# Twilight-Dream-Of-Magic/KolmogorovLike-DataCompressor

Hardware: AMD Instinct MI355X
Metric: compress MB/s at fixed block size, bit-exact vs reference; 1/2/4/8-GPU scaling (higher is better)
Workload: dtype u8; 1 GPU; enwik-style synthetic text (kolm.datagen.enwik_like, seed 20251212+rank), 256 MiB per GPU resident in HBM, 1 MiB fixed blocks, candidates 0..8 + MDL, payloads emitted in HBM; block_size=1048576, bytes_per_gpu=268435456, blocks_per_gpu=256, parallelism=block-shard x1

## Files before the change

### kolmogorovlike-datacompressor_amd/csrc/k_lsd.hip

```cpp
#include "kolm_internal.h"

#include <algorithm>
#include <cstdlib>
#include <string>
#include <vector>

namespace kolm {

namespace {

#ifndef KOLM_LSD_T
#define KOLM_LSD_T 4096
#endif
constexpr u32 LSD_T = KOLM_LSD_T;
constexpr u32 LSD_PT = LSD_T / WG;
static_assert(LSD_PT % 4 == 0 && LSD_PT <= 32, "head masks hold 32 slots per thread");

struct LsdGeom {
    Geom geo;
    u32 tpb;
    const u8* text;
    const u8* FEd;
    Factors fac;
    __device__ inline bool range(u32 t, u32& lo, u32& hi, u32& b) const {
        b = t / tpb;
        const u32 k = t - b * tpb;
        lo = geo.base(b) + k * LSD_T;
        const u32 e = geo.end(b);
        hi = min(lo + LSD_T, e);
        return lo < e;
    }
};

template <int P>
__device__ inline u32 digit(u32 key) {
    return (key >> (8 * P)) & 255u;
}

__device__ inline void load16(const u32* X, u32 i0, u32 hi, u32 (&v)[LSD_PT]) {
    if ((i0 & 3) == 0 && i0 + LSD_PT <= hi) {
        const uint4* p = reinterpret_cast<const uint4*>(X + i0);
#pragma unroll
        for (int q = 0; q < (int)LSD_PT / 4; ++q) {
            const uint4 t = p[q];
            v[4 * q] = t.x;
            v[4 * q + 1] = t.y;
            v[4 * q + 2] = t.z;
            v[4 * q + 3] = t.w;
        }
    } else {
#pragma unroll
        for (u32 e = 0; e < LSD_PT; ++e) v[e] = i0 + e < hi ? X[i0 + e] : 0u;
    }
// ... 505 lines not shown
    u32 len[LSD_PT];
    u32 nseg = 0;
#pragma unroll
    for (int e = LSD_PT - 1; e >= 0; --e) {
        const u32 i = i0 + e;
        len[e] = 0;
        if (hd[e]) {
            len[e] = nh - i;
            nh = i;
            nseg += len[e] >= 2;
        }
    }
    const u32 incl = wave_incl_scan(nseg, OpAddU(), 0u);
    if (lane == 63) sh3[w] = incl;
    if (split) anysplit = 1;
    __syncthreads();
    u32 off = incl - nseg;
    for (u32 q = 0; q < w; ++q) off += sh3[q];
    if (tid == WG - 1) {
        const u32 tot = off + nseg;
        wbase = tot ? atomicAdd(next_cnt, tot) : 0u;
        if (anysplit) blk_split[b] = 1;
    }
    __syncthreads();
    off += wbase;
#pragma unroll
    for (u32 e = 0; e < LSD_PT; ++e)
        if (len[e] >= 2) next[off++] = Seg{i0 + e, len[e]};
}

__global__ __launch_bounds__(WG) void k_r0_rk(Geom geo, u32 nwin, const u32* PP, u32* RK) {
    __shared__ u32 win[R0_WIN];
    const u32 b = blockIdx.x / nwin, k = blockIdx.x - b * nwin;
    const u32 base = geo.base(b), e = geo.end(b);
    const u32 lo = base + k * R0_WIN;
    if (lo >= e) return;
    const u32 n = min(R0_WIN, e - lo);
    for (u32 d = threadIdx.x; d < n; d += WG) {
        const u32 v = PP[lo + d];
        win[v >> 20] = base + (v & 0xFFFFFu);
    }
    __syncthreads();
    if ((lo & 3) == 0 && (n & 1023) == 0) {
        uint4* dst = reinterpret_cast<uint4*>(RK + lo);
        const uint4* src = reinterpret_cast<const uint4*>(win);
        for (u32 i = threadIdx.x; i < n / 4; i += WG) dst[i] = src[i];
    } else {
        for (u32 i = threadIdx.x; i < n; i += WG) RK[lo + i] = win[i];
    }
}

constexpr u32 AL_PER = 65536;

__global__ __launch_bounds__(WG) void k_alpha_present(Geom geo, const u8* text, u32 parts, u32* pres) {
    __shared__ u32 f[256];
    f[threadIdx.x] = 0;
    __syncthreads();
    const u32 b = blockIdx.x / parts, part = blockIdx.x - b * parts;
    const u32 lo = geo.base(b) + part * AL_PER, hi = min(lo + AL_PER, geo.end(b));
    for (u32 i = lo + threadIdx.x; i < hi; i += WG) f[text[i]] = 1u;
    __syncthreads();
    const u64 m = __ballot(f[threadIdx.x] != 0);
    if ((threadIdx.x & 31) == 0) {
        const u32 word = (u32)(m >> (threadIdx.x & 32));
        if (word) atomicOr(&pres[(u64)b * 8 + (threadIdx.x >> 5)], word);
    }
}

__global__ __launch_bounds__(WG) void k_alpha_codes(const u32* pres, u8* code, u32* wmax) {
    __shared__ u32 pw[8];
    const u32 b = blockIdx.x, c = threadIdx.x;
    if (c < 8) pw[c] = pres[(u64)b * 8 + c];
    __syncthreads();
    u32 r = 0;
    for (u32 k = 0; k < (c >> 5); ++k) r += __popc(pw[k]);
    r += __popc(pw[c >> 5] & ((1u << (c & 31)) - 1u));
    code[(u64)b * 256 + c] = (u8)r;
    if (c == 255) {
        const u32 sigma = r + ((pw[7] >> 31) & 1u);
        const u32 w = sigma > 1 ? 32 - __clz(sigma - 1) : 1u;
        atomicMax(wmax, w);
    }
}

__global__ __launch_bounds__(WG) void k_keypos_r0(LsdGeom g, const u8* code, u32 C, u32 w, u32 sh, u32* KA, u32* KB,
                                                  u32* hist0,
                                                  ScanParts sp = ScanParts{}, u32 part = 0) {
    __shared__ __align__(16) u8 tx[LSD_T + 64];
    __shared__ u8 cd[256];
    __shared__ TileCounts h0;
    u32 lo, hi, b;
    const u32 tile = xcd_tile();
    if (!g.range(tile, lo, hi, b)) {
        if (hist0) hist0[(u64)tile * 256 + threadIdx.x] = 0;
        return;
    }
    if (hist0) h0.clear();
    const u32 N = (u32)g.geo.N;
    cd[threadIdx.x] = code[(u64)b * 256 + threadIdx.x];
    const u32 n = min(hi + C + (part ? 1u : 0u), N) - lo;
    if ((((uintptr_t)g.text + lo) & 3) == 0) {
        const u32* src = reinterpret_cast<const u32*>(g.text + lo);
        u32* dst = reinterpret_cast<u32*>(tx);
        for (u32 i = threadIdx.x; i < (n + 3) / 4; i += WG) dst[i] = src[i];
    } else {
        for (u32 i = threadIdx.x; i < n; i += WG) tx[i] = g.text[lo + i];
    }
    __syncthreads();
    const u32 i0 = threadIdx.x * LSD_PT;
    if (lo + i0 < hi) {
    u8 fed[LSD_PT];
    if (((lo + i0) & 15) == 0 && lo + i0 + LSD_PT <= hi) {
#pragma unroll
        for (u32 q = 0; q < LSD_PT / 16; ++q) {
            const uint4 v = reinterpret_cast<const uint4*>(g.FEd + lo + i0)[q];
            const u32 wd[4] = {v.x, v.y, v.z, v.w};
#pragma unroll
            for (u32 e = 0; e < 16; ++e) fed[16 * q + e] = (u8)(wd[e >> 2] >> (8 * (e & 3)));
        }
    } else {
#pragma unroll
        for (u32 e = 0; e < LSD_PT; ++e) fed[e] = lo + i0 + e < hi ? g.FEd[lo + i0 + e] : (u8)255;
    }
    const u64 mask = C * w >= 64 ? ~0ull : ((1ull << (C * w)) - 1);
    u64 key = 0;
    for (u32 k = 0; k < C; ++k) key = (key << w) | (i0 + k < n ? cd[tx[i0 + k]] : 0u);
    u32 ka[LSD_PT], kb[LSD_PT];
    const u32 psh = w - part, plo = sh - part;
#pragma unroll
    for (u32 e = 0; e < LSD_PT; ++e) {
        const u32 x = i0 + e + C;
        const u32 nc = x < n ? cd[tx[x]] : 0u;
        const u64 kk = (key << sh) | (part ? (u64)(nc >> psh) << plo : 0ull);
        ka[e] = (u32)kk;
        kb[e] = (u32)(kk >> 32);
        key = ((key << w) | nc) & mask;
    }
    const u32 need = C + (part ? 1u : 0u);
#pragma unroll
    for (u32 e = 0; e < LSD_PT; ++e) {
        const u32 p = lo + i0 + e;
        if (p < hi && fed[e] < need) {
            u32 fs, m;
            g.fac.locate(g.geo, p, fs, m);
            u32 t = p - fs;
            u64 k2 = 0;
            for (u32 k = 0; k < C; ++k) {
                k2 = (k2 << w) | cd[g.text[fs + t]];
                if (++t == m) t = 0;
            }
            const u64 kk = (k2 << sh) | (part ? (u64)(cd[g.text[fs + t]] >> psh) << plo : 0ull);
            ka[e] = (u32)kk;
            kb[e] = (u32)(kk >> 32);
        }
    }
    const u32 p0 = lo + i0;
    if ((p0 & 3) == 0 && p0 + LSD_PT <= hi) {
#pragma unroll
        for (u32 q = 0; q < LSD_PT / 4; ++q) {
            reinterpret_cast<uint4*>(KA + p0)[q] = make_uint4(ka[4 * q], ka[4 * q + 1], ka[4 * q + 2], ka[4 * q + 3]);
            if (KB) reinterpret_cast<uint4*>(KB + p0)[q] = make_uint4(kb[4 * q], kb[4 * q + 1], kb[4 * q + 2], kb[4 * q + 3]);
        }
    } else {
        for (u32 e = 0; e < LSD_PT && p0 + e < hi; ++e) {
            KA[p0 + e] = ka[e];
            if (KB) KB[p0 + e] = kb[e];
        }
    }
    if (hist0) {
#pragma unroll
        for (u32 e = 0; e < LSD_PT; ++e)
            if (p0 + e < hi) h0.add(digit<0>(ka[e]));
    }
    }
    if (hist0) {
        __syncthreads();
        const u32 v = h0.total(threadIdx.x);
        hist0[(u64)tile * 256 + threadIdx.x] = v;
        add_part_total(g, sp, tile, v);
    }
}

template <int P, int SRC, int G, int OUT>
void lsd_pass(const LsdGeom& g, u32 nt, const u32* kin, const u32* pin, u32* kout, u32* pout, const u32* kg,
              u32* hist, bool counted, hipStream_t s, KTimer* kt, const ScanParts& sp) {
    static const std::string hn = "k_lsd_hist<" + std::to_string(P) + ", " + std::to_string(SRC) + ">";
    static const std::string sn = "k_lsd_scatter_w<" + std::to_string(P) + ", " + std::to_string(SRC) + ", " +
                                  std::to_string(G) + (OUT ? ", " + std::to_string(OUT) + ">" : std::string(">"));
    const u64 N = g.geo.N, H = (u64)nt * 1024;
    if (!counted) {
        KScope k(kt, KT_LSD, hn.c_str(), (SRC == SRC_REC ? 8 : 4) * N + H);
        k_lsd_hist<P, SRC><<<nt, WG, 0, s>>>(g, kin, hist, sp);
    }
    if (sp.cur) {
        KScope k(kt, KT_LSD, "k_lsd_scan2", 2 * H);
        k_lsd_scan2<<<g.geo.nb * sp.np, WG, 0, s>>>(g, hist, sp);
    } else {
        KScope k(kt, KT_LSD, "k_lsd_scan", 3 * H);
        static const int s4e = getenv("KOLM_LSD_SCAN4") ? atoi(getenv("KOLM_LSD_SCAN4")) : -1;
        const int mode = s4e >= 0 ? s4e : (g.geo.nb < 64 ? 1 : 0);
        if (mode == 1)
            k_lsd_scanp<4><<<g.geo.nb, 4 * WG, 0, s>>>(g, hist);
        else if (mode == 2)
            k_lsd_scanp<2><<<g.geo.nb, 2 * WG, 0, s>>>(g, hist);
        else
            k_lsd_scan<<<g.geo.nb, WG, 0, s>>>(g, hist);
    }
    {
        const u64 in = (SRC == SRC_PAIR || SRC == SRC_REC) ? 8 : 4, outb = OUT == OUT_PK ? 4 : 8;
        KScope k(kt, KT_LSD, sn.c_str(), (in + outb) * N + (G ? 4 * N : 0) + H);
        k_lsd_scatter_w<P, SRC, G, OUT><<<nt, WG, 0, s>>>(g, kin, pin, kout, pout, kg, hist);
    }
}

void run_pass_rec(u32 idx, const LsdGeom& g, u32 nt, const u32* kin, u32* kout, u32* pout, const u32* kg,
                  u32* hist, hipStream_t s, KTimer* kt, const ScanParts& sp) {
    switch (idx) {
        case 0: return lsd_pass<0, SRC_KP, 0, OUT_REC>(g, nt, kin, nullptr, kout, nullptr, nullptr, hist, true, s, kt, sp);
        case 1: return lsd_pass<1, SRC_REC, 0, OUT_REC>(g, nt, kin, nullptr, kout, nullptr, nullptr, hist, false, s, kt, sp);
        case 2: return lsd_pass<2, SRC_REC, 0, OUT_PK>(g, nt, kin, nullptr, kout, nullptr, nullptr, hist, false, s, kt, sp);
        case 3: return lsd_pass<3, SRC_PK, 1, OUT_REC>(g, nt, kin, nullptr, kout, nullptr, kg, hist, false, s, kt, sp);
        case 4: return lsd_pass<0, SRC_REC, 0, OUT_REC>(g, nt, kin, nullptr, kout, nullptr, nullptr, hist, false, s, kt, sp);
        case 5: return lsd_pass<1, SRC_REC, 0, OUT_REC>(g, nt, kin, nullptr, kout, nullptr, nullptr, hist, false, s, kt, sp);
        case 6: return lsd_pass<2, SRC_REC, 0, OUT_REC>(g, nt, kin, nullptr, kout, nullptr, nullptr, hist, false, s, kt, sp);
        default: return lsd_pass<3, SRC_REC, 0, OUT_PAIR>(g, nt, kin, nullptr, kout, pout, nullptr, hist, false, s, kt, sp);
    }
}

using PassFn = void (*)(const LsdGeom&, u32, const u32*, const u32*, u32*, u32*, const u32*, u32*, bool, hipStream_t,
                        KTimer*, const ScanParts&);
template <int P>
constexpr PassFn pass_of(int src_kp, int gat) {
    return src_kp ? (gat ? lsd_pass<P, SRC_KP, 1, 0> : lsd_pass<P, SRC_KP, 0, 0>)
                  : (gat ? lsd_pass<P, SRC_PAIR, 1, 0> : lsd_pass<P, SRC_PAIR, 0, 0>);
}
void run_pass(int P, bool src_kp, bool gat, const LsdGeom& g, u32 nt, const u32* kin, const u32* pin, u32* kout,
              u32* pout, const u32* kg, u32* hist, bool counted, hipStream_t s, KTimer* kt, int pk,
              const ScanParts& sp) {
    if (pk == 1) return lsd_pass<2, SRC_PAIR, 0, OUT_PK>(g, nt, kin, pin, kout, pout, kg, hist, counted, s, kt, sp);
    if (pk == 2) return lsd_pass<3, SRC_PK, 1, OUT_PAIR>(g, nt, kin, pin, kout, pout, kg, hist, counted, s, kt, sp);
    const int a = src_kp ? 1 : 0, c = gat ? 1 : 0;
    const PassFn f = P == 0 ? pass_of<0>(a, c) : P == 1 ? pass_of<1>(a, c) : P == 2 ? pass_of<2>(a, c) : pass_of<3>(a, c);
    f(g, nt, kin, pin, kout, pout, kg, hist, counted, s, kt, sp);
}

}

u32 lsd_tiles(const Geom& geo) { return (geo.bs + LSD_T - 1) / LSD_T * geo.nb; }

u32 launch_alpha(const Geom& geo, const u8* text, u32* pres, u8* code, u32* d_w, u32* h_w, bool compact,
                 hipStream_t s, KTimer* kt) {
    if (!geo.N) return 8;
    if (!compact) {
        std::vector<u8> id(256 * (size_t)geo.nb);
        for (size_t i = 0; i < id.size(); ++i) id[i] = (u8)i;
        KOLM_HIP_CHECK(hipMemcpyAsync(code, id.data(), id.size(), hipMemcpyHostToDevice, s));
        KOLM_HIP_CHECK(hipStreamSynchronize(s));
        return 8;
    }
    launch_alpha_async(geo, text, pres, code, d_w, h_w, s, kt);
    KOLM_HIP_CHECK(hipStreamSynchronize(s));
    return alpha_width(*h_w);
}

void launch_alpha_async(const Geom& geo, const u8* text, u32* pres, u8* code, u32* d_w, u32* h_w, hipStream_t s,
                        KTimer* kt, bool zeroed) {
    if (!geo.N) {
        if (h_w) *h_w = 8;
        return;
    }
    const u32 parts = (geo.bs + AL_PER - 1) / AL_PER;
    if (!zeroed) {
        KOLM_HIP_CHECK(hipMemsetAsync(pres, 0, sizeof(u32) * 8 * geo.nb, s));
        KOLM_HIP_CHECK(hipMemsetAsync(d_w, 0, sizeof(u32), s));
    }
    {
        KScope k(kt, KT_LSD, "k_alpha_present", geo.N);
        k_alpha_present<<<parts * geo.nb, WG, 0, s>>>(geo, text, parts, pres);
        k_alpha_codes<<<geo.nb, WG, 0, s>>>(pres, code, d_w);
    }
    if (h_w) KOLM_HIP_CHECK(hipMemcpyAsync(h_w, d_w, sizeof(u32), hipMemcpyDeviceToHost, s));
}

u32 alpha_width(u32 h_w) { return std::max<u32>(1, std::min<u32>(8, h_w)); }

void launch_round0(const Geom& geo, const R0Bufs& t, Seg* next, u32* next_cnt, u32* blk_split, hipStream_t s,
                   KTimer* kt) {
    if (!geo.N) return;
    LsdGeom g{geo, (geo.bs + LSD_T - 1) / LSD_T, t.text, t.FEd, t.fac};
    const u32 nt = g.tpb * geo.nb;
    const u64 N = geo.N;
    const u32 bits = t.chars * t.w, D = (bits + 7) / 8, sh = 8 * D - bits;
    const u32 pa = std::min<u32>(4, D), pb = D - pa;
    u32* K[2] = {t.K2, t.K22};
    u32* S[2] = {t.SA, t.SA2};
    const u32 T = pa + pb;
    int o = (T & 1) ? 0 : 1;
    {
        const u32 part = std::min(sh, t.w);
        const bool parts = t.swc && g.tpb > 1;
        ScanParts sp[2];
        if (parts) {
            u32 plt = 0;
            while (((g.tpb + (1u << plt) - 1) >> plt) > 16) ++plt;
            const u32 np = (g.tpb + (1u << plt) - 1) >> plt;
            const u64 cw = (u64)geo.nb * np * 256;
            sp[0] = ScanParts{t.swc, t.swc + cw, np, plt};
            sp[1] = ScanParts{t.swc + cw, t.swc, np, plt};
            KOLM_HIP_CHECK(hipMemsetAsync(t.swc, 0, sizeof(u32) * 2 * cw, s));
        }
        u32 pidx = 0;
        auto spp = [&]() -> const ScanParts& { return sp[parts ? (pidx & 1) : 0]; };
        {
            KScope k(kt, KT_KEYGEN, "k_keypos_r0", N * (pb ? 10 : 6));
            k_keypos_r0<<<nt, WG, 0, s>>>(g, t.code, t.chars, t.w, sh, t.RK, pb ? t.KP : nullptr, t.hist, spp(),
                                          part);
        }
        const bool pack = pa == 4 && pb > 0 && geo.bs <= (1u << 24);
        const bool rec = pack && pb == 4 && t.rec[0] && t.rec[1];
        if (rec) {
            u32* R2[2] = {reinterpret_cast<u32*>(t.rec[0]), reinterpret_cast<u32*>(t.rec[1])};
            const u32* in[8] = {t.RK, R2[0], R2[1], t.K22, R2[0], R2[1], R2[0], R2[1]};
            u32* out[8] = {R2[0], R2[1], t.K22, R2[0], R2[1], R2[0], R2[1], t.K2};
            for (u32 q = 0; q < 8; ++q, ++pidx)
                run_pass_rec(q, g, nt, in[q], out[q], q == 7 ? t.SA : nullptr, q == 3 ? t.KP : nullptr, t.hist, s, kt,
                             spp());
        }
        for (u32 q = 0; q < (rec ? 0u : pa); ++q) {
            const bool first = q == 0, gat = q + 1 == pa && pb > 0;
            const int pk = pack ? (q == 2 ? 1 : q == 3 ? 2 : 0) : 0;
            run_pass((int)q, first, gat, g, nt, first ? t.RK : K[o ^ 1], first ? nullptr : S[o ^ 1], K[o], S[o],
                     gat ? t.KP : nullptr, t.hist, first, s, kt, pk, spp());
            o ^= 1;
            ++pidx;
        }
        for (u32 q = 0; q < (rec ? 0u : pb); ++q) {
            run_pass((int)q, false, false, g, nt, K[o ^ 1], S[o ^ 1], K[o], S[o], nullptr, t.hist, false, s, kt, 0,
                     spp());
            o ^= 1;
            ++pidx;
        }
    }
    const bool win = geo.bs <= 256 * R0_WIN;
    {
        KScope k(kt, KT_LSD, "k_r0_tile_heads", (pb || win ? 12 : 4) * N);
        k_r0_tile_heads<<<nt, WG, 0, s>>>(g, t.K2, t.SA, pb ? t.RK : nullptr, t.HF, t.tmax, t.tmin,
                                          win ? t.hist : nullptr);
        k_tiles_max_scan<<<geo.nb, WG, 0, s>>>(t.tmax, t.cmax, g.tpb);
        k_r0_tiles_rscan<<<geo.nb, WG, 0, s>>>(t.tmin, t.cmin, g.tpb);
    }
    if (win) {
        const u32 nwin = (geo.bs + R0_WIN - 1) / R0_WIN;
        static const int s4e = getenv("KOLM_LSD_SCAN4") ? atoi(getenv("KOLM_LSD_SCAN4")) : -1;
        const int mode = s4e >= 0 ? s4e : (geo.nb < 64 ? 1 : 0);
        if (mode == 1)
            k_lsd_scanp<4><<<geo.nb, 4 * WG, 0, s>>>(g, t.hist);
        else if (mode == 2)
            k_lsd_scanp<2><<<geo.nb, 2 * WG, 0, s>>>(g, t.hist);
        else
            k_lsd_scan<<<geo.nb, WG, 0, s>>>(g, t.hist);
        {
            KScope k(kt, KT_LSD, "k_r0_final", 8 * N);
            k_r0_final<<<nt, WG, 0, s>>>(g, t.HF, t.SA, t.cmax, t.cmin, t.RK, next, next_cnt, blk_split, 0, 0, 1, 1, 0,
                                         t.hist, t.K22);
        }
        {
            KScope k(kt, KT_LSD, "k_r0_rk", 8 * N);
            k_r0_rk<<<nwin * geo.nb, WG, 0, s>>>(geo, nwin, t.K22, t.RK);
        }
// ... 15 lines not shown
```

### kolmogorovlike-datacompressor_amd/csrc/kolm_api.cpp

```cpp
#include <hip/hip_runtime.h>

#include <algorithm>
#include <atomic>
#include <chrono>
#include <sys/mman.h>
#include <condition_variable>
#include <cstdio>
#include <cstdlib>
#include <cstring>
#include <functional>
#include <map>
#include <memory>
#include <mutex>
#include <string>
#include <thread>
#include <vector>

#include "../../include/kolm.h"
#include "kolm_internal.h"

using namespace kolm;

namespace kolm {
thread_local std::string g_err;
// ... 379 lines not shown
    lv[0] = Level{c->get<LSeg>("lseg0", lseg_cap), cnt + C_L0SEG, c->get<LTile>("ltile0", ltile_cap), cnt + C_L0TILE,
                  cnt + C_L0ELEM};
    lv[1] = Level{c->get<LSeg>("lseg1", lseg_cap), cnt + C_L1SEG, c->get<LTile>("ltile1", ltile_cap), cnt + C_L1TILE,
                  cnt + C_L1ELEM};
    u32* hist = c->get<u32>("hist", ltile_cap * 256);

    if (!cyclic) {
        launch_iota(a.SA, N, s);
        launch_block_segs(segA, geo, s);
    }
    KOLM_HIP_CHECK(hipMemsetAsync(blk_done, 0, sizeof(u32) * geo.nb, s));
    if (cyclic) KOLM_HIP_CHECK(hipMemsetAsync(blk_last, 0, sizeof(u32) * geo.nb, s));
    Seg* cur = segA;
    Seg* nxt = segB;
    u32 ncur = geo.nb;
    u32 h0 = cyclic ? 8 : 3;
    const u32 kb_rank = bitlen(geo.bs) ? bitlen(geo.bs) : 1;
    u32* h = c->h_cnt;
    static const bool dbg = getenv("KOLM_DEBUG_ROUNDS") != nullptr;
    auto t_round = std::chrono::steady_clock::now();
    auto round_done = [&](u32 r) {
        if (!dbg) return;
        const auto now = std::chrono::steady_clock::now();
        fprintf(stderr, "[kolm] %s round %u: %.3f ms\n", cyclic ? "cyc" : "lin", r,
                std::chrono::duration<double, std::milli>(now - t_round).count());
        t_round = now;
    };
    constexpr int tiny_c = 4;
    int pend_done = -1;
    for (u32 round = 0; round < 64 && ncur; ++round) {
        a.initial = round == 0 ? 1 : 0;
        a.h = round == 0 ? 0u : (h0 << (round - 1));
        a.key_bits = a.initial ? (cyclic ? 32u : 27u) : bitlen(cyclic ? geo.bs - 1 : geo.bs);
        L.next = nxt;
        L.next_cnt = ncnt + (round & 1);
        const bool zero_bins = !(round == 0 && cyclic);
        {
            ZeroSpans z{};
            z.p[0] = L.next_cnt;
            z.n[0] = 1;
            z.p[1] = cnt;
            z.n[1] = C_STATUS;
            z.p[2] = cnt + C_CLSE;
            z.n[2] = C_N - C_CLSE;
            z.p[3] = a.blk_split;
            z.n[3] = (u32)geo.nb;
            if (pend_done >= 0) {
                z.done = blk_done;
                z.last = blk_last;
                z.round = (u32)pend_done;
                pend_done = -1;
            }
            if (round == 0 && cyclic && !alpha_ready) {
                z.p[4] = c->get<u32>("r0pres", (u64)geo.nb * 8);
                z.n[4] = (u32)geo.nb * 8;
            }
            if (zero_bins) {
                z.p[4] = c->get<u32>("cls_bins", NCLASS * CLS_NBIN);
                z.n[4] = NCLASS * CLS_NBIN;
                z.p[5] = c->get<u32>("cls_fill", NCLASS * CLS_NBIN);
                z.n[5] = NCLASS * CLS_NBIN;
            }
            launch_zero_spans(z, s);
        }
        if (round == 0 && cyclic) {
            const u64 nt = lsd_tiles(geo) + 1;
            u8* code = c->get<u8>("r0code", (u64)geo.nb * 256);
            u32 w;
            if (alpha_ready) {
                KOLM_HIP_CHECK(hipStreamWaitEvent(s, alpha_ready, 0));
                KOLM_HIP_CHECK(hipEventSynchronize(alpha_ready));
                w = alpha_width(h[H_ALPHA]);
            } else {
                launch_alpha_async(geo, text, c->get<u32>("r0pres", (u64)geo.nb * 8), code, cnt + C_ALPHA, nullptr,
                                   s, c->kt(), true);
                c->read_counts(h + C_ALPHA, cnt + C_ALPHA, 1, s);
                w = alpha_width(h[C_ALPHA]);
            }
            const u32 C = std::max<u32>(1, std::min<u32>(32, 64 / w));
            h0 = C;
            R0Bufs r{text, FEd, fac, code, C, w, c->get<u32>("KP", N), a.K2, a.SA, a.K22, a.SA2, a.RK,
                     c->get<u32>("r0hist", nt * 256), c->get<u32>("r0tmax", nt), c->get<u32>("r0tmin", nt),
                     c->get<u32>("r0cmax", nt), c->get<u32>("r0cmin", nt), c->get<u32>("r0hf", nt * WG),
                     c->get<u32>("r0swc", (u64)2 * geo.nb * 16 * 256)};
            r.rec[0] = c->get<u64>("r0rec0", N);
            r.rec[1] = c->get<u64>("r0rec1", N);
            out.r0_chars = C;
            if (dbg) fprintf(stderr, "[kolm] round 0: %u characters of %u bits\n", C, w);
            launch_round0(geo, r, nxt, L.next_cnt, a.blk_split, s, c->kt());
            out.active += N;
            out.rounds = 1;
            pend_done = 0;
            if (after_round0) {
                after_round0();
                c->active = s;
            }
            round_done(round);
            ncur = (u32)std::min<u64>(N / 2 + geo.nb, 0xFFFFFFFFu);
            ncur_dev = L.next_cnt;
            std::swap(cur, nxt);
            continue;
        }
        {
            TScope t(c, KOLM_KT_CLASSIFY, "k_classify", (u64)ncur * 24);
            const u32 nbits = bitlen((u32)(N - 1));
            const Bins bn{c->get<u32>("cls_bins", NCLASS * CLS_NBIN), c->get<u32>("cls_fill", NCLASS * CLS_NBIN),
                          nbits > 10 ? nbits - 10 : 0u};
            launch_classify_bins(cur, ncur, ncur_dev, a, L, lv[0], bn, s, zero_bins);
            a.xcd = 1;
        }
        c->read_counts(h, cnt, C_N, s);
        if (h[C_ACTIVE] == 0) break;
        out.active += h[C_ACTIVE];
        out.rounds = round + 1;
        if (dbg) {
            fprintf(stderr, "[kolm] round %u h=%u active=%u large: segs %u elems %u | class segs/elems:", round, a.h,
                    h[C_ACTIVE], h[C_L0SEG], h[C_L0ELEM]);
            for (int k = 0; k < NCLASS; ++k) fprintf(stderr, " %d:%u/%u", k, h[C_CLS + k], h[C_CLSE + k]);
            fprintf(stderr, "\n");
        }
        if (at_round) {
            at_round(round, cur, ncur, ncur_dev);
            c->active = s;
        }
        {
            a.KP = nullptr;
            constexpr u64 ddiv = 8;
            if ((u64)h[C_ACTIVE] * ddiv > N) {
                u32* KP = c->get<u32>("KP", N);
                TScope t(c, KOLM_KT_KEYGEN, "k_keypos", N * (cyclic ? 9 : 8));
                launch_keypos(a, KP, s);
                a.KP = KP;
            }
            const u64 per = a.KP ? 12 : a.initial ? (cyclic ? 20 : 11) : (cyclic ? 20 : 12);
            KgClasses kc{};
            u64 kg_elems = 0;
            for (int k = 1; k < NCLASS; ++k) {
                kc.segs[k] = L.cls[k];
                if (!h[C_CLS + k]) continue;
                if (a.KP && k <= tiny_c) continue;
                kc.count[k] = h[C_CLS + k];
// ... 358 lines not shown
    KOLM_HIP_CHECK(hipEventRecord(ev[0], ms));
    const bool want_rp = (mask >> KOLM_M_REPAIR) & 1u;
    RpArgs rpa{};
    if (want_rp) {
        rpa.geo = geo;
        rpa.text = d_text;
        rpa.ws_stride = repair_ws_bytes(bs);
        rpa.out_stride = 4ull * bs + 64;
        rpa.out = c->get<u8>("rp_out", (u64)nb * rpa.out_stride);
        rpa.result = c->get<u32>("rp_res", (u64)nb * RP_RS_N);
        static const bool rp_prof = getenv("KOLM_RP_PROF") && atoi(getenv("KOLM_RP_PROF")) != 0;
        if (rp_prof) {
            rpa.prof = c->get<u64>("rp_prof", (u64)nb * RP_P_N);
            KOLM_HIP_CHECK(hipMemsetAsync(rpa.prof, 0, sizeof(u64) * nb * RP_P_N, c->rp));
        }
        static const char* rp_trace = getenv("KOLM_RP_TRACE");
        if (rp_trace && *rp_trace) {
            rpa.trace = c->get<u32>("rp_trace", (u64)RP_TR_CAP * RP_TR_W);
            KOLM_HIP_CHECK(hipMemsetAsync(rpa.trace, 0, sizeof(u32) * RP_TR_CAP * RP_TR_W, c->rp));
        }
        u64 budget;
        if (getenv("KOLM_RP_WS_GB")) {
            budget = (u64)(atof(getenv("KOLM_RP_WS_GB")) * (double)(1ull << 30));
        } else {
            size_t fr = 0, total = 0;
            KOLM_HIP_CHECK(hipMemGetInfo(&fr, &total));
            const u64 held_rp = c->bytes_held("rp_ws");
            u64 held_other = 0;
            for (const auto& kv : c->bufs)
                if (kv.first != "rp_ws") held_other += kv.second.cap;
            const u64 need_other = 96 * N > held_other ? 96 * N - held_other : 0;
            const u64 avail = fr + held_rp > need_other ? fr + held_rp - need_other : 0;
            budget = (u64)(avail * 0.75);
        }
        const u32 group = (u32)std::max<u64>(1, std::min<u64>(nb, budget / rpa.ws_stride));
        rpa.ws = c->get<char>("rp_ws", (u64)group * rpa.ws_stride);
        KOLM_HIP_CHECK(hipStreamWaitEvent(c->rp, ev[0], 0));
        KOLM_HIP_CHECK(hipEventRecord(c->evr[1], c->rp));
        c->active = c->rp;
        for (u32 b0 = 0; b0 < nb; b0 += group) {
            const u32 k = std::min(group, nb - b0);
            TScope t(c, KOLM_KT_REPAIR, "k_repair", (u64)(geo.end(b0 + k - 1) - geo.base(b0)) * 9);
            launch_repair(rpa, b0, k, c->rp);
        }
        KOLM_HIP_CHECK(hipEventRecord(c->evr[0], c->rp));
    }
    KOLM_HIP_CHECK(hipStreamWaitEvent(s, ev[0], 0));
    c->active = s;
    P.lyndon();
    KOLM_HIP_CHECK(hipEventRecord(ev[5], s));
    static const int side_env = getenv("KOLM_SIDE_STREAM") ? atoi(getenv("KOLM_SIDE_STREAM")) : -1;
    const bool side = (side_env >= 0 ? side_env != 0 : nb < 64) && !serial && !want_rp;
    hipStream_t xs = side ? c->rp : ms;
    if (nb < 64) {
        c->active = xs;
        launch_alpha_async(geo, d_text, c->get<u32>("r0pres", (u64)nb * 8), c->get<u8>("r0code", (u64)nb * 256),
                           c->get<u32>("r0w", 1), c->h_cnt + H_ALPHA, xs, c->kt());
        KOLM_HIP_CHECK(hipEventRecord(c->eva, xs));
        P.alpha_ready = c->eva;
    }
    const bool want_lz = (mask >> KOLM_M_LZ77) & 1u || (h_force != nullptr);
    LzArgs z = P.lz_args();
    if (side) KOLM_HIP_CHECK(hipStreamWaitEvent(c->rp, ev[0], 0));
    c->active = xs;
    {
        EmitArgs ce{};
        ce.geo = geo;
        ce.text = d_text;
        ce.bits = d_bits;
        TScope t(c, KOLM_KT_SIZES, "k_cheap_sizes", N);
        launch_cheap_sizes(ce, xs);
    }
    const int prevc_idx = getenv("KOLM_PREVC_IDX") ? atoi(getenv("KOLM_PREVC_IDX")) : -1;
    if (!serial && (prevc_idx >= 0 ? prevc_idx != 0 : nb >= 16)) {
        KOLM_HIP_CHECK(hipStreamWaitEvent(xs, ev[5], 0));
        P.prevc();
        KOLM_HIP_CHECK(hipEventRecord(ev[6], xs));
        P.prevc_ready = ev[6];
    }
    if (side) KOLM_HIP_CHECK(hipEventRecord(ev[7], xs));
    c->active = ms;
    KOLM_HIP_CHECK(hipEventRecord(ej[0], ms));
    auto launch_lz = [&] {
        c->active = ms;
        KOLM_HIP_CHECK(hipEventRecord(ej[2], ms));
        if (want_lz) P.lz(z);
        KOLM_HIP_CHECK(hipEventRecord(ej[1], ms));
    };
    u8* bw = nullptr;
    P.early_gather = !serial && !want_rp;
    launch_lz();
    c->active = s;
    bw = P.cyclic();
    P.early_gather = false;
    KOLM_HIP_CHECK(hipMemcpyAsync(c->h_cnt + H_RSUM, c->get<u64>("rsum", 1), sizeof(u64), hipMemcpyDeviceToHost, s));
    KOLM_HIP_CHECK(hipEventRecord(ev[1], s));
    u8* mt = P.mtf(bw, d_bits);
    EmitArgs e{};
    e.geo = geo;
    e.text = d_text;
    e.mtf = mt;
    e.sizes = c->get<u32>("sizes", (u64)nb * KOLM_NCAND);
    e.bits = d_bits;
    e.method = c->get<u32>("method", nb);
    int32_t* d_force = nullptr;
    if (h_force) {
        d_force = c->get<int32_t>("force", nb);
        KOLM_HIP_CHECK(hipMemcpyAsync(d_force, h_force, sizeof(int32_t) * nb, hipMemcpyHostToDevice, s));
    }
    e.force = d_force;
    e.cand_mask = mask;
    e.off = c->get<u64>("off", nb + 1);
    e.arena = d_arena;
    e.arena_cap = arena_cap;
    const u64 ntiles = (u64)((geo.bs + TILE - 1) / TILE) * nb + 16;
    e.tile_tmp = c->get<u32>("tile_tmp", 2 * ntiles + 16);
// ... 1404 lines not shown
```

### kolmogorovlike-datacompressor_amd/csrc/kolm_internal.h

```cpp
#pragma once
#include <hip/hip_runtime.h>
#include <stdint.h>

#include <string>

namespace kolm {

void set_err(const std::string& s);

using u8 = uint8_t;
using u16 = uint16_t;
using u32 = uint32_t;
using u64 = uint64_t;

constexpr int TILE = 2048;
constexpr int WG = 256;
constexpr int PER_THREAD = TILE / WG;
constexpr int NCLASS = 12;
constexpr u32 NONE = 0xFFFFFFFFu;
constexpr int LZ_WINDOW = 4096;
constexpr int LZ_MIN = 3;
constexpr int LZ_CAP = 32;
constexpr int MTF_CHUNK = 1024;
constexpr u32 NCAND = 11;
// ... 233 lines not shown
void launch_med_sort(const LSeg* segs, u32 nseg, const u32* ndev, const SortArgs& a, const Lists& L,
                     hipStream_t s);
void launch_msd_hist(const LTile* tiles, u32 ntiles, const u32* ndev, const LSeg* segs, const SortArgs& a,
                     u32 shift, u32 width, u32* hist, hipStream_t s);
void launch_msd_scan(const LSeg* segs, u32 nseg, const u32* ndev, const SortArgs& a, u32 width, u32* hist,
                     bool last_level, const Lists& L, const Level& next, hipStream_t s);
void launch_msd_scatter(const LTile* tiles, u32 ntiles, const u32* ndev, const LSeg* segs, const SortArgs& a,
                        u32 shift, u32 width, const u32* hist, hipStream_t s);
void launch_copy_back(const LTile* tiles, u32 ntiles, const u32* ndev, const LSeg* segs, const SortArgs& a,
                      hipStream_t s);
constexpr int TINY_C = 5;
void launch_tiny_sort(int c, const Seg* segs, u32 count, const SortArgs& a, const Lists& L, hipStream_t s);
void launch_small_sort(int c, const Seg* segs, u32 count, const SortArgs& a, const Lists& L,
                       hipStream_t s);
struct SsClasses {
    const Seg* segs[NCLASS];
    u32 count[NCLASS];
    u32 wg0[NCLASS + 1];
};
void launch_small_sorts(SsClasses sc, bool w32, const SortArgs& a, const Lists& L, hipStream_t s);
void launch_finalize_eq(const Seg* eq, u32 count, const SortArgs& a, const Lists& L, hipStream_t s);
void launch_rounds_sum(const u32* blk_last, u32 nb, u64* out, hipStream_t s);
void launch_update_done(u32* blk_done, u32* blk_last, const u32* blk_split, u32 nb, u32 round, hipStream_t s);

u32 duval_span_bytes(const Geom& geo);
void launch_lyndon(const Geom& geo, const u8* text, u8* flag, u8* FEd, u32* fstart, uint4* fpre, u32* nfac,
                   u32* stack, u32* fcount, u32* tile_tmp, hipStream_t s, KTimer* kt = nullptr);
void launch_prevc(const Geom& geo, const u8* text, const u8* flag, Factors fac, u8* prevc, hipStream_t s);
void launch_bbwt_gather(const Geom& geo, const u32* SA, const u8* prevc, u8* out, hipStream_t s);
u32 bbwt_early_round();
void launch_mark_active(const Seg* cur, const u32* ncur_dev, u32 bound, u64* bm, hipStream_t s);
void launch_bbwt_gather_masked(const Geom& geo, const u32* SA, const u8* prevc, u8* out, const u64* bm,
                               hipStream_t s);

u32 lsd_tiles(const Geom& geo);
struct R0Bufs {
    const u8* text;
    const u8* FEd;
    Factors fac;
    const u8* code;
    u32 chars;
    u32 w;
    u32* KP;
    u32* K2;
    u32* SA;
    u32* K22;
    u32* SA2;
    u32* RK;
    u32* hist;
    u32 *tmax, *tmin, *cmax, *cmin;
    u32* HF;
    u32* swc = nullptr;
    u64* rec[2] = {nullptr, nullptr};
};
u32 launch_alpha(const Geom& geo, const u8* text, u32* pres, u8* code, u32* d_w, u32* h_w, bool compact,
                 hipStream_t s, KTimer* kt = nullptr);
void launch_alpha_async(const Geom& geo, const u8* text, u32* pres, u8* code, u32* d_w, u32* h_w, hipStream_t s,
                        KTimer* kt = nullptr, bool zeroed = false);
u32 alpha_width(u32 h_w);
void launch_round0(const Geom& geo, const R0Bufs& t, Seg* next, u32* next_cnt, u32* blk_split, hipStream_t s,
                   KTimer* kt = nullptr);



bool mtf_wave_mode(const Geom& geo);
u32 mtf_chunk_bytes(const Geom& geo);
u64 mtf_cp_words(const Geom& geo);
void launch_mtf(const Geom& geo, const u8* in, u8* out, u8* summary, u16* summary_cnt, u8* states,
                hipStream_t s, KTimer* kt = nullptr, u64* bits = nullptr, int rice_k = 2, u32* cp_scratch = nullptr);

struct EmitArgs {
    Geom geo;
    const u8* text;
    const u8* mtf;
    u32* sizes;
    u64* bits;
    u32* method;
    const int32_t* force;
    u32 cand_mask;
    u64* off;
    u8* arena;
    u64 arena_cap;
    u32* tile_tmp;
    u32* tile_tmp2;
    int rice_k;
};
void launch_cheap_sizes(const EmitArgs& e, hipStream_t s);
void launch_mdl(const EmitArgs& e, const u32* lz_sizes, const u32* rp_result, const u32* v2_size, u32* status,
                hipStream_t s);
void launch_emit_simple(const EmitArgs& e, hipStream_t s);
void launch_emit_rice(const EmitArgs& e, hipStream_t s);
void launch_rice_only(const Geom& geo, const u8* in, int k, u8* out, u32* tile_tmp, u32* tile_tmp2,
                      u32* out_size, hipStream_t s);

constexpr u32 V2_META = 11;
void launch_v2_sizes(const Geom& geo, const u8* text, u32* hist, u32* sel, u8* U, hipStream_t s,
                     KTimer* kt = nullptr);
void launch_v2_runs(u32 nplanes, const u32* d_pb, const u8* L, u64* rbits, u32* b1, hipStream_t s, KTimer* kt,
                    u64 bytes);
void launch_v2_size(const Geom& geo, const u32* sel, const u64* rbits, const u32* b1, u32* meta, u32* size,
                    hipStream_t s);
void launch_v2_emit(const Geom& geo, const u32* d_pb, const u32* meta, const u32* method, const u64* off,
                    const u8* U, const u8* L, u8* arena, hipStream_t s);

constexpr int LZL_HOME = 4096;
constexpr int LZL_CHUNK = 256;
constexpr int LZL_LEAD = 64;
constexpr int LZL_CAPX = 256;
constexpr u32 LZ_UNRES = 0x80000000u;

struct LzArgs {
    Geom geo;
// ... 141 lines not shown
```

Measured before the change: 8055 MB/s.

## Build frequency-weighted prefix codes for round-0 suffix sort keys

Samples per-block character frequencies in the alphabet kernel and builds a length-limited (2..8 bit) weighted prefix code per block on the GPU. A new round-0 key kernel packs each tile's text into a shared bitstream of variable-length codes and extracts 64-bit keys, so each key covers more characters than fixed-width alphabet codes when the alphabet needs more than 4 bits. The goal is to resolve more suffix ordering in round 0 and need fewer later doubling rounds, at the cost of a bitstream build with shared atomics, a slow fallback near factor ends, and extra weight buffers. It is enabled by default when the alphabet width exceeds 4 bits, which is likely for enwik-like text.

```diff
diff --git a/kolmogorovlike-datacompressor_amd/csrc/alpha_code.h b/kolmogorovlike-datacompressor_amd/csrc/alpha_code.h
--- /dev/null
+++ b/kolmogorovlike-datacompressor_amd/csrc/alpha_code.h
@@ -0,0 +1,99 @@
+#pragma once
+#include <cstdint>
+
+#if defined(__HIPCC__) || defined(__CUDACC__)
+#define AC_HD __host__ __device__
+#else
+#define AC_HD
+#endif
+
+namespace kolm {
+
+constexpr uint32_t AC_MAXLEN = 8;
+constexpr uint32_t AC_MINLEN = 2;
+constexpr uint32_t AC_KEYBITS = 64;
+constexpr uint32_t AC_R0_CHARS = AC_KEYBITS / AC_MAXLEN;
+constexpr uint32_t AC_MAXREAD = AC_KEYBITS / AC_MINLEN;
+constexpr uint32_t AC_NODES = 1u << (AC_MAXLEN + 1);
+
+struct AcWork {
+    uint64_t cum[257];
+    uint8_t sym[256];
+    uint16_t lo[AC_NODES];
+    uint16_t hi[AC_NODES];
+    uint32_t sigma;
+};
+
+AC_HD inline void ac_init(const uint32_t* pres, const uint32_t* wts, AcWork& k, uint16_t* cw) {
+    uint32_t n = 0;
+    uint64_t acc = 0;
+    k.cum[0] = 0;
+    for (uint32_t c = 0; c < 256; ++c) {
+        cw[c] = 0;
+        if ((pres[c >> 5] >> (c & 31)) & 1u) {
+            k.sym[n] = (uint8_t)c;
+            acc += wts[c] ? wts[c] : 1u;
+            k.cum[++n] = acc;
+        }
+    }
+    k.sigma = n;
+    for (uint32_t i = 0; i < AC_NODES; ++i) k.lo[i] = k.hi[i] = 0;
+    k.lo[1] = 0;
+    k.hi[1] = (uint16_t)n;
+}
+
+AC_HD inline void ac_node(AcWork& k, uint32_t id, uint32_t d, uint16_t* cw) {
+    const uint32_t lo = k.lo[id], hi = k.hi[id];
+    if (lo >= hi) return;
+    if (hi - lo == 1) {
+        const uint32_t len = d < AC_MINLEN ? AC_MINLEN : d;
+        const uint32_t code = (id - (1u << d)) << (len - d);
+        cw[k.sym[lo]] = (uint16_t)(len << 8 | code);
+        return;
+    }
+    if (d >= AC_MAXLEN) return;
+    const uint32_t cap = 1u << (AC_MAXLEN - d - 1);
+    const uint64_t base = k.cum[lo], tot = k.cum[hi] - base;
+    uint32_t a = lo + 1, b = hi;
+    while (a < b) {
+        const uint32_t m = (a + b) >> 1;
+        if (2 * (k.cum[m] - base) >= tot) b = m; else a = m + 1;
+    }
+    uint32_t s = a;
+    if (s > lo + 1) {
+        const uint64_t over = 2 * (k.cum[s] - base) - tot, under = tot - 2 * (k.cum[s - 1] - base);
+        if (under <= over) --s;
+    }
+    const uint32_t smin = hi - lo > cap ? hi - cap : lo + 1, smax = lo + cap < hi - 1 ? lo + cap : hi - 1;
+    if (s < smin) s = smin;
+    if (s > smax) s = smax;
+    k.lo[2 * id] = (uint16_t)lo;
+    k.hi[2 * id] = (uint16_t)s;
+    k.lo[2 * id + 1] = (uint16_t)s;
+    k.hi[2 * id + 1] = (uint16_t)hi;
+}
+
+AC_HD inline void ac_build(const uint32_t* pres, const uint32_t* wts, AcWork& k, uint16_t* cw) {
+    ac_init(pres, wts, k, cw);
+    for (uint32_t d = 0; d <= AC_MAXLEN; ++d)
+        for (uint32_t id = 1u << d; id < (2u << d); ++id) ac_node(k, id, d, cw);
+}
+
+AC_HD inline uint32_t ac_len(uint16_t w) { return w >> 8; }
+AC_HD inline uint32_t ac_bits(uint16_t w) { return w & 255u; }
+
+AC_HD inline uint64_t ac_key_wrap(const uint8_t* text, uint32_t m, uint32_t t, const uint16_t* cw) {
+    uint64_t key = 0;
+    uint32_t nb = 0;
+    for (uint32_t k = 0; k < AC_MAXREAD && nb < AC_KEYBITS; ++k) {
+        const uint16_t w = cw[text[t]];
+        const uint32_t l = ac_len(w), room = AC_KEYBITS - nb;
+        if (!l) break;
+        key |= l <= room ? (uint64_t)ac_bits(w) << (room - l) : (uint64_t)ac_bits(w) >> (l - room);
+        nb += l;
+        if (++t == m) t = 0;
+    }
+    return key;
+}
+
+}
diff --git a/kolmogorovlike-datacompressor_amd/csrc/k_lsd.hip b/kolmogorovlike-datacompressor_amd/csrc/k_lsd.hip
--- a/kolmogorovlike-datacompressor_amd/csrc/k_lsd.hip
+++ b/kolmogorovlike-datacompressor_amd/csrc/k_lsd.hip
@@ -1,4 +1,5 @@
 #include "kolm_internal.h"
+#include "alpha_code.h"
 
 #include <algorithm>
 #include <cstdlib>
@@ -610,23 +611,32 @@
 
 constexpr u32 AL_PER = 65536;
 
-__global__ __launch_bounds__(WG) void k_alpha_present(Geom geo, const u8* text, u32 parts, u32* pres) {
+__global__ __launch_bounds__(WG) void k_alpha_weights(Geom geo, const u8* text, u32 parts, u32* pres, u32* wts) {
     __shared__ u32 f[256];
+    __shared__ u32 cn[256];
     f[threadIdx.x] = 0;
+    cn[threadIdx.x] = 0;
     __syncthreads();
     const u32 b = blockIdx.x / parts, part = blockIdx.x - b * parts;
-    const u32 lo = geo.base(b) + part * AL_PER, hi = min(lo + AL_PER, geo.end(b));
-    for (u32 i = lo + threadIdx.x; i < hi; i += WG) f[text[i]] = 1u;
+    const u32 base = geo.base(b), lo = base + part * AL_PER, hi = min(lo + AL_PER, geo.end(b));
+    for (u32 i = lo + threadIdx.x; i < hi; i += WG) {
+        const u32 c = text[i];
+        f[c] = 1u;
+        if (wts && ((i - base) & 0xF0u) == 0) atomicAdd(&cn[c], 1u);
+    }
     __syncthreads();
     const u64 m = __ballot(f[threadIdx.x] != 0);
     if ((threadIdx.x & 31) == 0) {
         const u32 word = (u32)(m >> (threadIdx.x & 32));
         if (word) atomicOr(&pres[(u64)b * 8 + (threadIdx.x >> 5)], word);
     }
-}
-
-__global__ __launch_bounds__(WG) void k_alpha_codes(const u32* pres, u8* code, u32* wmax) {
+    if (wts && cn[threadIdx.x]) atomicAdd(&wts[(u64)b * 256 + threadIdx.x], cn[threadIdx.x]);
+}
+
+__global__ __launch_bounds__(WG) void k_alpha_codes(const u32* pres, const u32* wts, u8* code, u16* cw, u32* wmax) {
     __shared__ u32 pw[8];
+    __shared__ AcWork ak;
+    __shared__ u16 cws[256];
     const u32 b = blockIdx.x, c = threadIdx.x;
     if (c < 8) pw[c] = pres[(u64)b * 8 + c];
     __syncthreads();
@@ -634,11 +644,38 @@
     for (u32 k = 0; k < (c >> 5); ++k) r += __popc(pw[k]);
     r += __popc(pw[c >> 5] & ((1u << (c & 31)) - 1u));
     code[(u64)b * 256 + c] = (u8)r;
+    const bool here = (pw[c >> 5] >> (c & 31)) & 1u;
     if (c == 255) {
-        const u32 sigma = r + ((pw[7] >> 31) & 1u);
+        const u32 sigma = r + (here ? 1u : 0u);
         const u32 w = sigma > 1 ? 32 - __clz(sigma - 1) : 1u;
         atomicMax(wmax, w);
     }
+    if (!cw) return;
+    cws[c] = 0;
+    for (u32 i = c; i < AC_NODES; i += WG) ak.lo[i] = ak.hi[i] = 0;
+    if (here) {
+        ak.sym[r] = (u8)c;
+        const u32 v = wts[(u64)b * 256 + c];
+        ak.cum[r + 1] = v ? v : 1u;
+    }
+    __syncthreads();
+    if (c == 255) {
+        const u32 sigma = r + (here ? 1u : 0u);
+        u64 acc = 0;
+        ak.cum[0] = 0;
+        for (u32 i = 1; i <= sigma; ++i) {
+            acc += ak.cum[i];
+            ak.cum[i] = acc;
+        }
+        ak.sigma = sigma;
+        ak.hi[1] = (u16)sigma;
+    }
+    __syncthreads();
+    for (u32 d = 0; d <= AC_MAXLEN; ++d) {
+        if (c < (1u << d)) ac_node(ak, (1u << d) + c, d, cws);
+        __syncthreads();
+    }
+    cw[(u64)b * 256 + c] = cws[c];
 }
 
 __global__ __launch_bounds__(WG) void k_keypos_r0(LsdGeom g, const u8* code, u32 C, u32 w, u32 sh, u32* KA, u32* KB,
@@ -737,6 +774,141 @@
         hist0[(u64)tile * 256 + threadIdx.x] = v;
         add_part_total(g, sp, tile, v);
     }
+}
+
+constexpr u32 R0C_TAIL = AC_MAXREAD;
+constexpr u32 R0C_WORDS = (LSD_T + R0C_TAIL) * AC_MAXLEN / 32 + 4;
+__global__ __launch_bounds__(WG) void k_keypos_r0c(LsdGeom g, const u16* cwt, u32* KA, u32* KB, u32* hist0,
+                                                   ScanParts sp) {
+    __shared__ __align__(16) u8 tx[LSD_T + 64];
+    __shared__ u16 cw[256];
+    __shared__ u32 bs[R0C_WORDS];
+    __shared__ u32 wsum[WG / 64];
+    __shared__ TileCounts h0;
+    u32 lo, hi, b;
+    const u32 tile = xcd_tile(), tid = threadIdx.x, lane = tid & 63, wv = tid >> 6;
+    if (!g.range(tile, lo, hi, b)) {
+        hist0[(u64)tile * 256 + tid] = 0;
+        return;
+    }
+    h0.clear();
+    const u32 N = (u32)g.geo.N;
+    cw[tid] = cwt[(u64)b * 256 + tid];
+    for (u32 i = tid; i < R0C_WORDS; i += WG) bs[i] = 0;
+    const u32 n = min(hi + R0C_TAIL, N) - lo;
+    if ((((uintptr_t)g.text + lo) & 3) == 0) {
+        const u32* src = reinterpret_cast<const u32*>(g.text + lo);
+        u32* dst = reinterpret_cast<u32*>(tx);
+        for (u32 i = tid; i < (n + 3) / 4; i += WG) dst[i] = src[i];
+    } else {
+        for (u32 i = tid; i < n; i += WG) tx[i] = g.text[lo + i];
+    }
+    __syncthreads();
+    const u32 i0 = tid * LSD_PT;
+    u32 mine = 0;
+#pragma unroll
+    for (u32 e = 0; e < LSD_PT; ++e) mine += i0 + e < n ? ac_len(cw[tx[i0 + e]]) : 0u;
+    const u32 incl = wave_incl_scan(mine, OpAddU(), 0u);
+    if (lane == 63) wsum[wv] = incl;
+    __syncthreads();
+    u32 off = incl - mine, total = 0;
+#pragma unroll
+    for (u32 q = 0; q < WG / 64; ++q) {
+        off += q < wv ? wsum[q] : 0u;
+        total += wsum[q];
+    }
+    {
+        u32 o = off, wi = o >> 5, cur = 0;
+#pragma unroll
+        for (u32 e = 0; e < LSD_PT; ++e) {
+            const u16 v = i0 + e < n ? cw[tx[i0 + e]] : (u16)0;
+            const u32 l = ac_len(v), c = ac_bits(v), s = o & 31;
+            if (l) {
+                if (s + l < 32) {
+                    cur |= c << (32 - s - l);
+                } else {
+                    const u32 r = s + l - 32;
+                    atomicOr(&bs[wi], cur | (c >> r));
+                    ++wi;
+                    cur = r ? c << (32 - r) : 0u;
+                }
+                o += l;
+            }
+        }
+        if (cur) atomicOr(&bs[wi], cur);
+    }
+    if (wv == 0) {
+        const u32 x = LSD_T + lane;
+        const u16 v = lane < R0C_TAIL && x < n ? cw[tx[x]] : (u16)0;
+        const u32 l = ac_len(v), c = ac_bits(v);
+        const u32 o = total + wave_incl_scan(l, OpAddU(), 0u) - l, s = o & 31;
+        if (l) {
+            if (s + l <= 32) {
+                atomicOr(&bs[o >> 5], c << (32 - s - l));
+            } else {
+                const u32 r = s + l - 32;
+                atomicOr(&bs[o >> 5], c >> r);
+                atomicOr(&bs[(o >> 5) + 1], c << (32 - r));
+            }
+        }
+    }
+    __syncthreads();
+    if (lo + i0 < hi) {
+        u8 fed[LSD_PT];
+        if (((lo + i0) & 15) == 0 && lo + i0 + LSD_PT <= hi) {
+#pragma unroll
+            for (u32 q = 0; q < LSD_PT / 16; ++q) {
+                const uint4 v = reinterpret_cast<const uint4*>(g.FEd + lo + i0)[q];
+                const u32 wd[4] = {v.x, v.y, v.z, v.w};
+#pragma unroll
+                for (u32 e = 0; e < 16; ++e) fed[16 * q + e] = (u8)(wd[e >> 2] >> (8 * (e & 3)));
+            }
+        } else {
+#pragma unroll
+            for (u32 e = 0; e < LSD_PT; ++e) fed[e] = lo + i0 + e < hi ? g.FEd[lo + i0 + e] : (u8)255;
+        }
+        u32 ka[LSD_PT], kb[LSD_PT];
+        u32 o = off;
+#pragma unroll
+        for (u32 e = 0; e < LSD_PT; ++e) {
+            const u32 wi = o >> 5, s = o & 31;
+            const u32 w0 = bs[wi], w1 = bs[wi + 1], w2 = bs[wi + 2];
+            kb[e] = __funnelshift_l(w1, w0, s);
+            ka[e] = __funnelshift_l(w2, w1, s);
+            o += i0 + e < n ? ac_len(cw[tx[i0 + e]]) : 0u;
+        }
+#pragma unroll
+        for (u32 e = 0; e < LSD_PT; ++e) {
+            const u32 p = lo + i0 + e;
+            if (p < hi && fed[e] <= AC_MAXREAD) {
+                u32 fs, m;
+                g.fac.locate(g.geo, p, fs, m);
+                const u64 kk = ac_key_wrap(g.text + fs, m, p - fs, cw);
+                ka[e] = (u32)kk;
+                kb[e] = (u32)(kk >> 32);
+            }
+        }
+        const u32 p0 = lo + i0;
+        if ((p0 & 3) == 0 && p0 + LSD_PT <= hi) {
+#pragma unroll
+            for (u32 q = 0; q < LSD_PT / 4; ++q) {
+                reinterpret_cast<uint4*>(KA + p0)[q] = make_uint4(ka[4 * q], ka[4 * q + 1], ka[4 * q + 2], ka[4 * q + 3]);
+                reinterpret_cast<uint4*>(KB + p0)[q] = make_uint4(kb[4 * q], kb[4 * q + 1], kb[4 * q + 2], kb[4 * q + 3]);
+            }
+        } else {
+            for (u32 e = 0; e < LSD_PT && p0 + e < hi; ++e) {
+                KA[p0 + e] = ka[e];
+                KB[p0 + e] = kb[e];
+            }
+        }
+#pragma unroll
+        for (u32 e = 0; e < LSD_PT; ++e)
+            if (p0 + e < hi) h0.add(digit<0>(ka[e]));
+    }
+    __syncthreads();
+    const u32 v = h0.total(tid);
+    hist0[(u64)tile * 256 + tid] = v;
+    add_part_total(g, sp, tile, v);
 }
 
 template <int P, int SRC, int G, int OUT>
@@ -816,31 +988,40 @@
         KOLM_HIP_CHECK(hipStreamSynchronize(s));
         return 8;
     }
-    launch_alpha_async(geo, text, pres, code, d_w, h_w, s, kt);
+    launch_alpha_async(geo, text, pres, code, nullptr, d_w, h_w, s, kt);
     KOLM_HIP_CHECK(hipStreamSynchronize(s));
     return alpha_width(*h_w);
 }
 
-void launch_alpha_async(const Geom& geo, const u8* text, u32* pres, u8* code, u32* d_w, u32* h_w, hipStream_t s,
-                        KTimer* kt, bool zeroed) {
+void launch_alpha_async(const Geom& geo, const u8* text, u32* pres, u8* code, u16* cw, u32* d_w, u32* h_w,
+                        hipStream_t s, KTimer* kt, bool zeroed) {
     if (!geo.N) {
         if (h_w) *h_w = 8;
         return;
     }
     const u32 parts = (geo.bs + AL_PER - 1) / AL_PER;
     if (!zeroed) {
-        KOLM_HIP_CHECK(hipMemsetAsync(pres, 0, sizeof(u32) * 8 * geo.nb, s));
+        KOLM_HIP_CHECK(hipMemsetAsync(pres, 0, sizeof(u32) * alpha_pres_words(geo.nb, cw != nullptr), s));
         KOLM_HIP_CHECK(hipMemsetAsync(d_w, 0, sizeof(u32), s));
     }
     {
-        KScope k(kt, KT_LSD, "k_alpha_present", geo.N);
-        k_alpha_present<<<parts * geo.nb, WG, 0, s>>>(geo, text, parts, pres);
-        k_alpha_codes<<<geo.nb, WG, 0, s>>>(pres, code, d_w);
+        u32* wts = cw ? pres + (u64)8 * geo.nb : nullptr;
+        KScope k(kt, KT_LSD, "k_alpha_weights", geo.N);
+        k_alpha_weights<<<parts * geo.nb, WG, 0, s>>>(geo, text, parts, pres, wts);
+        k_alpha_codes<<<geo.nb, WG, 0, s>>>(pres, wts, code, cw, d_w);
     }
     if (h_w) KOLM_HIP_CHECK(hipMemcpyAsync(h_w, d_w, sizeof(u32), hipMemcpyDeviceToHost, s));
 }
 
 u32 alpha_width(u32 h_w) { return std::max<u32>(1, std::min<u32>(8, h_w)); }
+
+u64 alpha_pres_words(u32 nb, bool weights) { return (u64)nb * (weights ? 8 + 256 : 8); }
+
+bool r0_code_mode(u32 w) {
+    if (getenv("KOLM_R0_CODE")) return atoi(getenv("KOLM_R0_CODE")) != 0;
+    return w > 4;
+}
+u32 r0_code_chars() { return AC_R0_CHARS; }
 
 void launch_round0(const Geom& geo, const R0Bufs& t, Seg* next, u32* next_cnt, u32* blk_split, hipStream_t s,
                    KTimer* kt) {
@@ -870,9 +1051,12 @@
         u32 pidx = 0;
         auto spp = [&]() -> const ScanParts& { return sp[parts ? (pidx & 1) : 0]; };
         {
-            KScope k(kt, KT_KEYGEN, "k_keypos_r0", N * (pb ? 10 : 6));
-            k_keypos_r0<<<nt, WG, 0, s>>>(g, t.code, t.chars, t.w, sh, t.RK, pb ? t.KP : nullptr, t.hist, spp(),
-                                          part);
+            KScope k(kt, KT_KEYGEN, t.cw ? "k_keypos_r0c" : "k_keypos_r0", N * (pb ? 10 : 6));
+            if (t.cw)
+                k_keypos_r0c<<<nt, WG, 0, s>>>(g, t.cw, t.RK, t.KP, t.hist, spp());
+            else
+                k_keypos_r0<<<nt, WG, 0, s>>>(g, t.code, t.chars, t.w, sh, t.RK, pb ? t.KP : nullptr, t.hist, spp(),
+                                              part);
         }
         const bool pack = pa == 4 && pb > 0 && geo.bs <= (1u << 24);
         const bool rec = pack && pb == 4 && t.rec[0] && t.rec[1];
diff --git a/kolmogorovlike-datacompressor_amd/csrc/kolm_api.cpp b/kolmogorovlike-datacompressor_amd/csrc/kolm_api.cpp
--- a/kolmogorovlike-datacompressor_amd/csrc/kolm_api.cpp
+++ b/kolmogorovlike-datacompressor_amd/csrc/kolm_api.cpp
@@ -455,8 +455,8 @@
                 pend_done = -1;
             }
             if (round == 0 && cyclic && !alpha_ready) {
-                z.p[4] = c->get<u32>("r0pres", (u64)geo.nb * 8);
-                z.n[4] = (u32)geo.nb * 8;
+                z.p[4] = c->get<u32>("r0pres", alpha_pres_words(geo.nb, true));
+                z.n[4] = (u32)alpha_pres_words(geo.nb, true);
             }
             if (zero_bins) {
                 z.p[4] = c->get<u32>("cls_bins", NCLASS * CLS_NBIN);
@@ -469,18 +469,21 @@
         if (round == 0 && cyclic) {
             const u64 nt = lsd_tiles(geo) + 1;
             u8* code = c->get<u8>("r0code", (u64)geo.nb * 256);
+            u16* cw = c->get<u16>("r0cw", (u64)geo.nb * 256);
             u32 w;
             if (alpha_ready) {
                 KOLM_HIP_CHECK(hipStreamWaitEvent(s, alpha_ready, 0));
                 KOLM_HIP_CHECK(hipEventSynchronize(alpha_ready));
                 w = alpha_width(h[H_ALPHA]);
             } else {
-                launch_alpha_async(geo, text, c->get<u32>("r0pres", (u64)geo.nb * 8), code, cnt + C_ALPHA, nullptr,
-                                   s, c->kt(), true);
+                launch_alpha_async(geo, text, c->get<u32>("r0pres", alpha_pres_words(geo.nb, true)), code, cw,
+                                   cnt + C_ALPHA, nullptr, s, c->kt(), true);
                 c->read_counts(h + C_ALPHA, cnt + C_ALPHA, 1, s);
                 w = alpha_width(h[C_ALPHA]);
             }
-            const u32 C = std::max<u32>(1, std::min<u32>(32, 64 / w));
+            const bool codes = r0_code_mode(w);
+            if (codes) w = 8;
+            const u32 C = codes ? r0_code_chars() : std::max<u32>(1, std::min<u32>(32, 64 / w));
             h0 = C;
             R0Bufs r{text, FEd, fac, code, C, w, c->get<u32>("KP", N), a.K2, a.SA, a.K22, a.SA2, a.RK,
                      c->get<u32>("r0hist", nt * 256), c->get<u32>("r0tmax", nt), c->get<u32>("r0tmin", nt),
@@ -488,8 +491,11 @@
                      c->get<u32>("r0swc", (u64)2 * geo.nb * 16 * 256)};
             r.rec[0] = c->get<u64>("r0rec0", N);
             r.rec[1] = c->get<u64>("r0rec1", N);
+            r.cw = codes ? cw : nullptr;
             out.r0_chars = C;
-            if (dbg) fprintf(stderr, "[kolm] round 0: %u characters of %u bits\n", C, w);
+            if (dbg)
+                fprintf(stderr, "[kolm] round 0: %u characters of %u bits%s\n", C, w,
+                        codes ? " (prefix codes, 64 key bits)" : "");
             launch_round0(geo, r, nxt, L.next_cnt, a.blk_split, s, c->kt());
             out.active += N;
             out.rounds = 1;
@@ -954,16 +960,17 @@
     static const int side_env = getenv("KOLM_SIDE_STREAM") ? atoi(getenv("KOLM_SIDE_STREAM")) : -1;
     const bool side = (side_env >= 0 ? side_env != 0 : nb < 64) && !serial && !want_rp;
     hipStream_t xs = side ? c->rp : ms;
+    if (side) KOLM_HIP_CHECK(hipStreamWaitEvent(c->rp, ev[0], 0));
     if (nb < 64) {
         c->active = xs;
-        launch_alpha_async(geo, d_text, c->get<u32>("r0pres", (u64)nb * 8), c->get<u8>("r0code", (u64)nb * 256),
+        launch_alpha_async(geo, d_text, c->get<u32>("r0pres", alpha_pres_words(nb, true)),
+                           c->get<u8>("r0code", (u64)nb * 256), c->get<u16>("r0cw", (u64)nb * 256),
                            c->get<u32>("r0w", 1), c->h_cnt + H_ALPHA, xs, c->kt());
         KOLM_HIP_CHECK(hipEventRecord(c->eva, xs));
         P.alpha_ready = c->eva;
     }
     const bool want_lz = (mask >> KOLM_M_LZ77) & 1u || (h_force != nullptr);
     LzArgs z = P.lz_args();
-    if (side) KOLM_HIP_CHECK(hipStreamWaitEvent(c->rp, ev[0], 0));
     c->active = xs;
     {
         EmitArgs ce{};
diff --git a/kolmogorovlike-datacompressor_amd/csrc/kolm_internal.h b/kolmogorovlike-datacompressor_amd/csrc/kolm_internal.h
--- a/kolmogorovlike-datacompressor_amd/csrc/kolm_internal.h
+++ b/kolmogorovlike-datacompressor_amd/csrc/kolm_internal.h
@@ -309,12 +309,16 @@
     u32* HF;
     u32* swc = nullptr;
     u64* rec[2] = {nullptr, nullptr};
+    const u16* cw = nullptr;
 };
 u32 launch_alpha(const Geom& geo, const u8* text, u32* pres, u8* code, u32* d_w, u32* h_w, bool compact,
                  hipStream_t s, KTimer* kt = nullptr);
-void launch_alpha_async(const Geom& geo, const u8* text, u32* pres, u8* code, u32* d_w, u32* h_w, hipStream_t s,
-                        KTimer* kt = nullptr, bool zeroed = false);
+void launch_alpha_async(const Geom& geo, const u8* text, u32* pres, u8* code, u16* cw, u32* d_w, u32* h_w,
+                        hipStream_t s, KTimer* kt = nullptr, bool zeroed = false);
 u32 alpha_width(u32 h_w);
+u64 alpha_pres_words(u32 nb, bool weights);
+bool r0_code_mode(u32 w);
+u32 r0_code_chars();
 void launch_round0(const Geom& geo, const R0Bufs& t, Seg* next, u32* next_cnt, u32* blk_split, hipStream_t s,
                    KTimer* kt = nullptr);
 
```

Result: faster. 8373 MB/s (median of 6 runs) (+3.9%).
